# nfurnon/disco

Hardware: NVIDIA H100
Metric: beamformed frames/sec (16kHz, 512-pt STFT) (higher is better)
Workload: dtype f32 (c64 spectra, f32 SCM accumulation, f64 per-bin solve)

## Files before the change

### disco_b200/csrc/common.cuh

```cuda
#pragma once
#include <cuda_runtime.h>
#include <stdint.h>

#define DISCO_DEV __device__ __forceinline__

namespace disco {

DISCO_DEV float2 fadd2(float2 a, float2 b) { return make_float2(__fadd_rn(a.x, b.x), __fadd_rn(a.y, b.y)); }
DISCO_DEV float2 fmul2(float2 a, float2 b) { return make_float2(__fmul_rn(a.x, b.x), __fmul_rn(a.y, b.y)); }
DISCO_DEV float2 ffma2(float2 a, float2 b, float2 c) {
    return make_float2(__fmaf_rn(a.x, b.x, c.x), __fmaf_rn(a.y, b.y, c.y));
}

DISCO_DEV double solve_scale(double t) {
    if (!(t >= 2.2250738585072014e-308 && t <= 1.7976931348623157e308)) return 1.0;
    const int e = ((__double2hiint(t) >> 20) & 0x7ff) - 1023;
    return __hiloint2double((1023 - e) << 20, 0);
}

DISCO_DEV float2 cadd(float2 a, float2 b) { return fadd2(a, b); }
DISCO_DEV float2 csub(float2 a, float2 b) { return fadd2(a, make_float2(-b.x, -b.y)); }
DISCO_DEV float2 cmul(float2 a, float2 b) {
    const float2 t = fmul2(make_float2(-b.y, b.x), make_float2(a.y, a.y));
    return ffma2(b, make_float2(a.x, a.x), t);
}
DISCO_DEV float2 cmulc(float2 a, float2 b) {
    const float2 t = fmul2(make_float2(a.y, -a.x), make_float2(b.y, b.y));
    return ffma2(a, make_float2(b.x, b.x), t);
}
DISCO_DEV float2 cfma(float2 a, float2 b, float2 acc) {
    const float2 t = ffma2(b, make_float2(a.x, a.x), acc);
    return ffma2(make_float2(-b.y, b.x), make_float2(a.y, a.y), t);
}
DISCO_DEV float2 cfma_cj(float2 a, float2 b, float2 acc) {
    const float2 t = ffma2(b, make_float2(a.x, a.x), acc);
    return ffma2(make_float2(b.y, -b.x), make_float2(a.y, a.y), t);
}
DISCO_DEV float2 cscale(float2 a, float s) { return fmul2(a, make_float2(s, s)); }
DISCO_DEV float2 cconj(float2 a) { return make_float2(a.x, -a.y); }
DISCO_DEV float2 cfma_r(float s, float2 a, float2 acc) { return ffma2(make_float2(s, s), a, acc); }

template <int C>
DISCO_DEV void dual_filter(const float2 (&w1)[C], const float2 (&w2)[C], const float2 (&y)[C], int ref, float2& z,
                           float2& zn, float2& yf) {
    z = make_float2(0.f, 0.f);
    yf = make_float2(0.f, 0.f);
#pragma unroll
    for (int c = 0; c < C; ++c) {
        z = cfma_cj(w1[c], y[c], z);
        yf = cfma_cj(w2[c], y[c], yf);
    }
    float2 r = y[0];
#pragma unroll
    for (int c = 1; c < C; ++c)
        if (c == ref) r = y[c];
    zn = csub(r, z);
}

DISCO_DEV uint32_t smem_u32(const void* p) { return (uint32_t)__cvta_generic_to_shared(p); }

DISCO_DEV void mbar_init(uint64_t* bar, uint32_t count) {
    asm volatile("mbarrier.init.shared::cta.b64 [%0], %1;" ::"r"(smem_u32(bar)), "r"(count));
}
DISCO_DEV void mbar_expect_tx(uint64_t* bar, uint32_t bytes) {
    asm volatile("mbarrier.arrive.expect_tx.shared::cta.b64 _, [%0], %1;" ::"r"(smem_u32(bar)), "r"(bytes)
                 : "memory");
}
DISCO_DEV void mbar_arrive(uint64_t* bar) {
    asm volatile("mbarrier.arrive.shared::cta.b64 _, [%0];" ::"r"(smem_u32(bar)) : "memory");
}
DISCO_DEV void mbar_wait(uint64_t* bar, uint32_t parity) {
    const uint32_t addr = smem_u32(bar);
    uint32_t done;
    do {
        asm volatile(
            "{\n"
            ".reg .pred p;\n"
            "mbarrier.try_wait.parity.shared::cta.b64 p, [%1], %2, %3;\n"
            "selp.u32 %0, 1, 0, p;\n"
            "}\n"
            : "=r"(done)
            : "r"(addr), "r"(parity), "r"(20000u)
            : "memory");
    } while (!done);
}
DISCO_DEV void tma_load_1d(void* dst_smem, const void* src_gmem, uint32_t bytes, uint64_t* bar) {
    asm volatile(
        "cp.async.bulk.shared::cluster.global.mbarrier::complete_tx::bytes [%0], [%1], %2, [%3];" ::"r"(
            smem_u32(dst_smem)),
        "l"(src_gmem), "r"(bytes), "r"(smem_u32(bar))
        : "memory");
}
DISCO_DEV void named_bar_sync(int id, int nthreads) {
    asm volatile("bar.sync %0, %1;" ::"r"(id), "r"(nthreads) : "memory");
}
DISCO_DEV void fence_proxy_async() { asm volatile("fence.proxy.async.shared::cta;" ::: "memory"); }
DISCO_DEV void fence_mbar_init() { asm volatile("fence.mbarrier_init.release.cluster;" ::: "memory"); }

DISCO_DEV void st_stream(float2* p, float2 v) { __stcs(p, v); }
DISCO_DEV float ld_stream(const float* p) { return __ldcs(p); }
DISCO_DEV float2 ld_stream(const float2* p) { return __ldcs(p); }

}
```

### disco_b200/csrc/stft_scm.cu

```cuda
#include "common.cuh"
#include "kernels.h"
#include "stft_core.cuh"

namespace disco {

enum : int { OUT_Y = 0, OUT_NONE = 1, OUT_FILTER = 2, OUT_FILTER_FT = 3 };

template <int N, int C, int NM = 1, int OUT = OUT_Y>
struct StftCfg : StftJob<N> {
    static constexpr bool WIDE = C > 4;
    static constexpr int NSTG = 2;
    static constexpr int JOBS = 8;
    static constexpr int ITEMS = JOBS * StftJob<N>::NB;
    static constexpr int P = (C + 1) / 2;
    static constexpr int TT = ITEMS / P;
    static constexpr bool REALLOC = (N == 512) || (WIDE && N == 256);
    static constexpr bool DEAL = N == 512 && NM == 2 && C >= 3 && !WIDE;
    static constexpr int FFT_WARPS = DEAL ? 7 : (N == 512 && (WIDE || NM == 2)) ? 4 : 8;
    static constexpr int JPW = JOBS / FFT_WARPS;
    static constexpr int FFT_ARRIVALS = DEAL ? JOBS : FFT_WARPS;
    static constexpr int SCM_WARPS = N / 64;
    static constexpr int LEAD_WARPS = (REALLOC && !DEAL) ? 4 : 1;
    static constexpr int WARPS = LEAD_WARPS + FFT_WARPS + SCM_WARPS;
    static constexpr int THREADS = 32 * WARPS;
    static constexpr int SPEC = ITEMS * StftJob<N>::ROWP;
    static constexpr int SAMP = C * (TT + 1) * StftJob<N>::H;
    static constexpr int REG_LAUNCH = 16384 / ((WARPS + 3) / 4) / 32 / 8 * 8;
    static constexpr bool FILT = OUT == OUT_FILTER || OUT == OUT_FILTER_FT;
    static constexpr int REG_SCM = FILT ? 80 : WIDE ? 184 : ((N == 512 && NM == 2) ? 152 : 120);
    static constexpr int REG_FFT_CAP = 256;
    static constexpr int REG_ALLOC = (REG_LAUNCH > 255 ? 255 : REG_LAUNCH) * THREADS;
    static constexpr int REG_LEAD_OWN = FILT ? 56 : 32;
    static constexpr int REG_FFT_LEFT =
        DEAL ? (REG_ALLOC - 32 * SCM_WARPS * REG_SCM) / (32 * (LEAD_WARPS + FFT_WARPS)) / 8 * 8
             : (REG_ALLOC - 128 * REG_LEAD_OWN - 32 * SCM_WARPS * REG_SCM) / (32 * FFT_WARPS) / 8 * 8;
    static constexpr int REG_FFT = REG_FFT_LEFT < REG_FFT_CAP ? REG_FFT_LEFT : REG_FFT_CAP;
    static constexpr int REG_LEAD = DEAL ? REG_FFT : REG_LEAD_OWN;
    static constexpr int REG_SUM = DEAL ? 32 * (LEAD_WARPS + FFT_WARPS) * REG_FFT + 32 * SCM_WARPS * REG_SCM
                                        : 128 * REG_LEAD + 32 * FFT_WARPS * REG_FFT + 32 * SCM_WARPS * REG_SCM;
    static constexpr int FT_PITCH = 34;
    static constexpr int FT_STAGE = OUT == OUT_FILTER_FT ? SCM_WARPS * 8 * FT_PITCH : 0;
    static_assert(!REALLOC || (REG_LEAD >= 24 && REG_FFT >= 24), "setmaxnreg budgets start at 24");
    static_assert(!REALLOC || REG_SUM <= (REG_LAUNCH > 255 ? 255 : REG_LAUNCH) * THREADS,
                  "register budgets exceed the CTA's allocation");
    static_assert(!DEAL || (REALLOC && LEAD_WARPS + FFT_WARPS == 8 && WARPS == 16 && REG_LAUNCH == 128 &&
                            REG_FFT == 104 && REG_SUM == 65536),
                  "DEAL: loader + 7 FFT warps fill two warpgroups at 104 registers next to 8 SCM warps at 152");
    static_assert(DEAL || WIDE || NM != 2 || N != 512 || (FFT_WARPS == 4 && REG_SCM == 152 && REG_FFT == 176),
                  "two masks, 1-2 microphones at 512 points: 4 FFT warps at 176 registers next to SCM warps at 152");
    static_assert(!DEAL || JOBS >= FFT_WARPS, "DEAL: every FFT warp must run a job of every tile (the fill barrier)");
};

int stft_tile_frames(int n_fft, int C) { return (8 * (32 / (n_fft / 32))) / ((C + 1) / 2); }

template <int N, int C, int OUT = OUT_Y>
__host__ __device__ inline size_t smem_bytes() {
    using G = StftCfg<N, C, 1, OUT>;
    return G::NSTG * ((size_t)G::SPEC * sizeof(float2) + (size_t)G::SAMP * sizeof(float)) + (size_t)N * sizeof(float2) + 256 +
           64 * sizeof(float) + (size_t)G::FT_STAGE * sizeof(float2);
}

__device__ __forceinline__ long long range_lo(long long total, int b, int nb) { return total * b / nb; }

template <int R, int LAUNCH>
DISCO_DEV void set_maxnreg() {
    if constexpr (R > LAUNCH) {
        asm volatile("setmaxnreg.inc.sync.aligned.u32 %0;\n" ::"n"(R));
    } else if constexpr (R < LAUNCH) {
        asm volatile("setmaxnreg.dec.sync.aligned.u32 %0;\n" ::"n"(R));
    }
}

template <int C, int NM>
struct ScmAcc {
    static constexpr int NOFF = C * (C - 1) / 2;
    static constexpr int NO = NOFF > 0 ? NOFF : 1;
    float2 d[NM > 0 ? NM : 1][C];
    float2 os[NM > 0 ? NM : 1][NO];
    float2 on[NM > 0 ? NM : 1][NO];
    DISCO_DEV void reset() {
#pragma unroll
        for (int q = 0; q < NM; ++q) {
#pragma unroll
            for (int i = 0; i < C; ++i) d[q][i] = make_float2(0.f, 0.f);
#pragma unroll
            for (int i = 0; i < NOFF; ++i) os[q][i] = on[q][i] = make_float2(0.f, 0.f);
        }
    }
    DISCO_DEV void step(const float2 (&y)[C], const float (&m)[NM > 0 ? NM : 1]) {
        float2 ab[NM > 0 ? NM : 1];
#pragma unroll
        for (int q = 0; q < NM; ++q) {
            const float om = 1.f - m[q];
            ab[q] = make_float2(m[q] * m[q], om * om);
        }
        int o = 0;
#pragma unroll
        for (int i = 0; i < C; ++i) {
            const float dd = fmaf(y[i].x, y[i].x, y[i].y * y[i].y);
#pragma unroll
            for (int q = 0; q < NM; ++q) d[q][i] = ffma2(make_float2(dd, dd), ab[q], d[q][i]);
#pragma unroll
            for (int j = i + 1; j < C; ++j) {
                const float2 op = cmulc(y[i], y[j]);
#pragma unroll
                for (int q = 0; q < NM; ++q) {
                    os[q][o] = cfma_r(ab[q].x, op, os[q][o]);
                    on[q][o] = cfma_r(ab[q].y, op, on[q][o]);
                }
                ++o;
            }
        }
    }
    DISCO_DEV void flush(float* out, int F) const {
        int a = 0;
#pragma unroll
        for (int q = 0; q < NM; ++q) {
#pragma unroll
            for (int i = 0; i < C; ++i) out[(size_t)(a++) * F] = d[q][i].x;
#pragma unroll
            for (int i = 0; i < NOFF; ++i) {
                out[(size_t)(a++) * F] = os[q][i].x;
                out[(size_t)(a++) * F] = os[q][i].y;
            }
#pragma unroll
            for (int i = 0; i < C; ++i) out[(size_t)(a++) * F] = d[q][i].y;
#pragma unroll
            for (int i = 0; i < NOFF; ++i) {
                out[(size_t)(a++) * F] = on[q][i].x;
                out[(size_t)(a++) * F] = on[q][i].y;
            }
        }
    }
};

enum : int { RC_SAMP_FULL = 0, RC_SAMP_EMPTY = 1, RC_SPEC_FULL = 2, RC_SPEC_EMPTY = 3 };
enum : int { RC_ROLE_LOADER = 1, RC_ROLE_FFT = 2, RC_ROLE_SCM = 3 };
#ifdef DISCO_ROLE_CLOCKS
constexpr int RC_MAX_CTAS = 1024, RC_SLOTS = 8;
__device__ unsigned long long g_role_clocks[RC_MAX_CTAS * 32 * RC_SLOTS];
DISCO_DEV long long rc_clock() {
    long long t;
    asm volatile("mov.u64 %0, %%clock64;" : "=l"(t)::"memory");
    return t;
}
struct RoleClocks {
    long long t0, w[4] = {0, 0, 0, 0};
    int tiles = 0, jobs = 0;
    DISCO_DEV RoleClocks() : t0(rc_clock()) {}
    DISCO_DEV void wait(int k, uint64_t* bar, uint32_t parity) {
        const long long a = rc_clock();
        mbar_wait(bar, parity);
        w[k] += rc_clock() - a;
    }
    DISCO_DEV void tile() { ++tiles; }
    DISCO_DEV void job() { ++jobs; }
    DISCO_DEV void done(int role) {
        const long long t1 = rc_clock();
        if ((threadIdx.x & 31) != 0 || blockIdx.x >= RC_MAX_CTAS) return;
        unsigned long long* o = g_role_clocks + ((size_t)blockIdx.x * 32 + (threadIdx.x >> 5)) * RC_SLOTS;
        o[0] = role;
        o[1] = tiles;
        o[2] = jobs;
        o[3] = t1 - t0;
        for (int k = 0; k < 4; ++k) o[4 + k] = w[k];
    }
};
#else
struct RoleClocks {
    DISCO_DEV void wait(int, uint64_t* bar, uint32_t parity) { mbar_wait(bar, parity); }
    DISCO_DEV void tile() {}
    DISCO_DEV void job() {}
    DISCO_DEV void done(int) {}
};
#endif

template <int OUT>
struct StftParam {
    using type = StftArgs;
};
template <>
struct StftParam<OUT_FILTER> {
    using type = StftFilterArgs;
};
template <>
struct StftParam<OUT_FILTER_FT> {
    using type = StftFilterArgs;
};

template <int N, int C, int NM, int OUT>
__global__ void __launch_bounds__(StftCfg<N, C, NM, OUT>::THREADS, 1) stft_scm_kernel(typename StftParam<OUT>::type p) {
    using G = StftCfg<N, C, NM, OUT>;
    constexpr int RA = G::RA, NB = G::NB, H = G::H, F = G::F, ROWP = G::ROWP, P = G::P, TT = G::TT;
    constexpr int SAMP = G::SAMP;
    constexpr int NACC = NM * 2 * C * C;
    constexpr int NMX = NM > 0 ? NM : 1;
    constexpr bool SCM = NM > 0;
    constexpr bool STORE_Y = OUT == OUT_Y, FILT = G::FILT, FT = OUT == OUT_FILTER_FT;
    static_assert(!FILT || NM == 0, "the filter consumer accumulates no statistics");
    constexpr int MCAP = (G::REALLOC && G::REG_SCM >= 152 && !G::WIDE) ? 16 : 8;
    constexpr int MC = (TT * NM <= MCAP) ? TT : ((MCAP / NMX) < TT ? (MCAP / NMX) : TT);
    constexpr int NCH = (TT + MC - 1) / MC;

    extern __shared__ __align__(128) unsigned char smem_raw[];
    constexpr int NSTG = G::NSTG;
    float2* spec = reinterpret_cast<float2*>(smem_raw);
    float* samp = reinterpret_cast<float*>(spec + NSTG * G::SPEC);
    float2* tw = reinterpret_cast<float2*>(samp + NSTG * SAMP);
    uint64_t* bars = reinterpret_cast<uint64_t*>(tw + N);
    uint64_t* samp_full = bars;
    uint64_t* samp_empty = bars + NSTG;
    uint64_t* spec_full = bars + 2 * NSTG;
    uint64_t* spec_empty = bars + 3 * NSTG;
    float* nyq = reinterpret_cast<float*>(bars + 32);
    float2* ft_stage = reinterpret_cast<float2*>(nyq + 64);
    static_assert(4 * NSTG <= 32, "barrier area");
    static_assert(TT * C <= 64 && TT <= 32, "Nyquist staging");

    const int tid = threadIdx.x, lane = tid & 31, warp = tid >> 5;
    const int L = p.L, T = p.T;
    const int tiles_per_grp = (T + TT - 1) / TT;
    const long long total = (long long)p.n_grp * tiles_per_grp;
    const long long lo = range_lo(total, blockIdx.x, gridDim.x), hi = range_lo(total, blockIdx.x + 1, gridDim.x);
    const int n_it = (int)(hi - lo);
    if (n_it <= 0) return;

    for (int i = tid; i < N; i += blockDim.x) tw[i] = p.twiddle[i];
    if (tid == 0) {
        for (int s = 0; s < NSTG; ++s) {
            mbar_init(&samp_full[s], 1);
            mbar_init(&samp_empty[s], G::FFT_ARRIVALS);
            mbar_init(&spec_full[s], G::FFT_ARRIVALS);
            mbar_init(&spec_empty[s], G::SCM_WARPS + 1);
        }
        fence_mbar_init();
    }
    __syncthreads();

    auto tile_of = [&](int it, int& grp, int& t0) {
        const long long i = lo + it;
        grp = (int)(i / tiles_per_grp);
        t0 = (int)(i % tiles_per_grp) * TT;
    };
    auto seg_slot = [&](int grp) { return blockIdx.x - seg_slots(grp, tiles_per_grp, total, gridDim.x).first; };
    auto mask_at = [&](int q, int grp, int t, int f) {
        const float* m = q == 0 ? p.mask : p.mask2;
        return p.mask_ft ? m[((size_t)grp * F + f) * T + t] : m[((size_t)grp * T + t) * F + f];
    };

    constexpr int FFT_WARP0 = G::LEAD_WARPS;
    constexpr int SCM_WARP0 = G::LEAD_WARPS + G::FFT_WARPS;
    const bool is_fft = warp >= FFT_WARP0 && warp < FFT_WARP0 + G::FFT_WARPS;
    if constexpr (G::DEAL) {
        if (warp < SCM_WARP0) set_maxnreg<G::REG_FFT, G::REG_LAUNCH>();
    }
    if (warp < G::LEAD_WARPS) {
        if (G::REALLOC && !G::DEAL) set_maxnreg<G::REG_LEAD, G::REG_LAUNCH>();
        if (warp != 0) return;
        RoleClocks rc;
        auto load_tile = [&](int it) {
            int grp, t0;
            tile_of(it, grp, t0);
            const int nfr = min(TT, T - t0), s = it % NSTG, c_valid = min(C, p.n_sig - grp * C);
            rc.wait(RC_SAMP_EMPTY, &samp_empty[s], ((it / NSTG) & 1) ^ 1);
            const float* xg = p.x + (size_t)grp * C * L;
            float* dst = samp + s * SAMP;
            const int s0 = t0 * H - H;
            const int cnt = (nfr + 1) * H;
            const int k_lo = max(0, -s0), k_hi = min(cnt, L - s0);
            if (lane == 0) {
                if (p.use_tma && k_hi > k_lo) {
                    fence_proxy_async();
                    mbar_expect_tx(&samp_full[s], (uint32_t)(c_valid * (k_hi - k_lo) * sizeof(float)));
                    for (int c = 0; c < c_valid; ++c)
                        tma_load_1d(dst + c * (TT + 1) * H + k_lo, xg + (size_t)c * L + s0 + k_lo,
                                    (uint32_t)((k_hi - k_lo) * sizeof(float)), &samp_full[s]);
                } else {
                    mbar_arrive(&samp_full[s]);
                }
            }
        };
        constexpr int NP = C * (C + 1) / 2;
        constexpr int NSLOT = NP > 32 ? 2 : 1;
        int pi[NSLOT], pj[NSLOT], row[NSLOT];
#pragma unroll
        for (int u = 0; u < NSLOT; ++u) {
            const int pp = min(lane + 32 * u, NP - 1);
            if (pp < C) {
                pi[u] = pj[u] = pp;
                row[u] = pp;
            } else {
                int o = pp - C, i = 0, n = C - 1;
                while (o >= n) {
                    o -= n;
                    --n;
                    ++i;
                }
                pi[u] = i;
                pj[u] = i + 1 + o;
                row[u] = C + 2 * (pp - C);
            }
        }
        float as[NMX][NSLOT], an[NMX][NSLOT];
        auto nyq_reset = [&]() {
#pragma unroll
            for (int q = 0; q < NMX; ++q)
#pragma unroll
                for (int u = 0; u < NSLOT; ++u) as[q][u] = an[q][u] = 0.f;
        };
        nyq_reset();
        float2 nw1[FILT ? C : 1], nw2[FILT ? C : 1];
        int nw_grp = -1;
        for (int i = 0; i < NSTG - 1; ++i)
            if (i < n_it) load_tile(i);
        for (int it = 0; it < n_it; ++it) {
            if (it + NSTG - 1 < n_it) load_tile(it + NSTG - 1);
            int grp, t0;
            tile_of(it, grp, t0);
            const int nfr = min(TT, T - t0), s = it % NSTG, c_valid = min(C, p.n_sig - grp * C);
            if constexpr (FILT) {
                if (grp != nw_grp) {
#pragma unroll
                    for (int c = 0; c < C; ++c) {
                        nw1[c] = p.W1[((size_t)grp * F + F - 1) * C + c];
                        nw2[c] = p.W2[((size_t)grp * F + F - 1) * C + c];
                    }
                    nw_grp = grp;
                }
                rc.wait(RC_SPEC_FULL, &spec_full[s], (it / NSTG) & 1);
                if (lane < nfr) {
                    float2 y[C];
#pragma unroll
                    for (int c = 0; c < C; ++c) {
                        const float2 z = spec[s * G::SPEC + (size_t)(lane * P + c / 2) * ROWP + N / 2];
                        y[c] = make_float2(stft_nyquist(z, c & 1), 0.f);
                    }
                    float2 z, zn, yf;
                    dual_filter<C>(nw1, nw2, y, p.ref, z, zn, yf);
                    const size_t o = FT ? ((size_t)grp * F + F - 1) * T + t0 + lane : ((size_t)grp * T + t0 + lane) * F + (F - 1);
                    __stcs(p.z + o, z);
                    if (p.zn) __stcs(p.zn + o, zn);
                    __stcs(p.yf + o, yf);
                }
                __syncwarp();
                if (lane == 0) mbar_arrive(&spec_empty[s]);
            } else {
                float mq[NMX];
#pragma unroll
                for (int q = 0; q < NMX; ++q) mq[q] = (SCM && lane < nfr) ? mask_at(q, grp, t0 + lane, F - 1) : 0.f;
                rc.wait(RC_SPEC_FULL, &spec_full[s], (it / NSTG) & 1);
#pragma unroll
                for (int r = lane; r < TT * C; r += 32) {
                    const int tl_l = r / C, c_l = r % C;
                    float yv = 0.f;
                    if (tl_l < nfr && c_l < c_valid) {
                        const float2 z = spec[s * G::SPEC + (size_t)(tl_l * P + c_l / 2) * ROWP + N / 2];
                        yv = (c_l & 1) ? z.y + z.y : z.x + z.x;
                        if (STORE_Y) p.Y[(((size_t)grp * C + c_l) * T + t0 + tl_l) * F + (F - 1)] = make_float2(yv, 0.f);
                    }
                    nyq[r] = yv;
                }
                __syncwarp();
                if (lane == 0) mbar_arrive(&spec_empty[s]);
                if (SCM) {
#pragma unroll
                    for (int tl = 0; tl < TT; ++tl) {
                        if (tl < nfr) {
                            float pr[NSLOT];
#pragma unroll
                            for (int u = 0; u < NSLOT; ++u)
                                pr[u] = nyq[tl * C + pi[u]] * nyq[tl * C + pj[u]];
#pragma unroll
                            for (int q = 0; q < NM; ++q) {
                                const float m = __shfl_sync(0xffffffffu, mq[q], tl), om = 1.f - m;
                                const float a = m * m, b = om * om;
#pragma unroll
                                for (int u = 0; u < NSLOT; ++u) {
                                    as[q][u] = fmaf(a, pr[u], as[q][u]);
                                    an[q][u] = fmaf(b, pr[u], an[q][u]);
                                }
                            }
                        }
                    }
                    const bool seg_end = (it + 1 == n_it) || ((lo + it + 1) % tiles_per_grp == 0);
                    if (seg_end) {
                        float* out = p.part + ((size_t)grp * p.slots_per_grp + seg_slot(grp)) * NACC * F + (F - 1);
#pragma unroll
                        for (int u = 0; u < NSLOT; ++u) {
                            const int pp = lane + 32 * u;
                            if (pp < NP) {
#pragma unroll
                                for (int q = 0; q < NM; ++q) {
                                    float* os = out + (size_t)(q * 2 * C * C) * F;
                                    float* on = os + (size_t)(C * C) * F;
                                    os[(size_t)row[u] * F] = as[q][u];
                                    on[(size_t)row[u] * F] = an[q][u];
                                    if (pp >= C) {
                                        os[(size_t)(row[u] + 1) * F] = 0.f;
                                        on[(size_t)(row[u] + 1) * F] = 0.f;
                                    }
                                }
                            }
                        }
                        nyq_reset();
                    }
                }
                __syncwarp();
            }
            rc.tile();
        }
        rc.done(RC_ROLE_LOADER);
    } else if (is_fft) {
        if (G::REALLOC && !G::DEAL) set_maxnreg<G::REG_FFT, G::REG_LAUNCH>();
        const int wf = warp - FFT_WARP0, f0 = wf / G::FFT_WARPS, w = wf % G::FFT_WARPS;
        constexpr bool WINREG = (RA <= 16);
        float win[WINREG ? RA : 1];
        if (WINREG) {
#pragma unroll
            for (int j = 0; j < RA; ++j) win[j] = p.window[lane + 32 * j];
        }
        RoleClocks rc;
        struct FftTile {
            int s, nfr, c_valid;
            const float* sm;
            bool full;
        };
        auto enter_tile = [&](int it) {
            int grp, t0;
            tile_of(it, grp, t0);
            const int nfr = min(TT, T - t0), s = it % NSTG, c_valid = min(C, p.n_sig - grp * C);
            const uint32_t ph = (it / NSTG) & 1;
            const float* sm = samp + s * SAMP;
            rc.wait(RC_SAMP_FULL, &samp_full[s], ph);
            {
                const int s0 = t0 * H - H;
                const int cnt = (nfr + 1) * H;
                int k_lo = max(0, -s0), k_hi = min(cnt, L - s0);
                if (!p.use_tma || k_hi <= k_lo) k_lo = k_hi = 0;
                const int n_fill = cnt - (k_hi - k_lo);
                if (n_fill > 0) {
                    const float* xg = p.x + (size_t)grp * C * L;
                    float* dst = samp + s * SAMP;
                    named_bar_sync(1 + f0, 32 * G::FFT_WARPS);
                    for (int c = 0; c < c_valid; ++c)
#pragma unroll(G::DEAL ? 1 : 4)
                        for (int q = w * 32 + lane; q < n_fill; q += 32 * G::FFT_WARPS) {
                            const int k = q < k_lo ? q : q + (k_hi - k_lo);
                            const int sidx = reflect_index(s0 + k, L);
                            float v = 0.f;
                            if (sidx >= 0 && sidx < L) v = xg[(size_t)c * L + sidx];
                            dst[c * (TT + 1) * H + k] = v;
                        }
                    named_bar_sync(1 + f0, 32 * G::FFT_WARPS);
                }
            }
            rc.wait(RC_SPEC_EMPTY, &spec_empty[s], ph ^ 1);
            const bool full = (nfr == TT && c_valid == C && (C % 2 == 0) && (G::ITEMS % P == 0));
            return FftTile{s, nfr, c_valid, sm, full};
        };
        auto run_job = [&](const FftTile& tc, int jb, bool release) {
            const int s = tc.s, nfr = tc.nfr, c_valid = tc.c_valid;
            const float* sm = tc.sm;
            const bool full = tc.full;
            float2* job = spec + s * G::SPEC + (size_t)jb * NB * ROWP;
            constexpr bool TWREG = (RA <= 16);
            float2 twr[TWREG ? RA : 1];
            if (TWREG) {
#pragma unroll
                for (int k1 = 1; k1 < RA; ++k1) twr[k1] = tw[k1 * 32 + lane];
            }
#pragma unroll
            for (int q = 0; q < NB; ++q) {
                const int item = jb * NB + q;
                const int tl = item / P, pr = item % P;
                const int ca = 2 * pr, cb = 2 * pr + 1;
                const float* xa = sm + ca * (TT + 1) * H + tl * H + lane;
                const float* xb = sm + cb * (TT + 1) * H + tl * H + lane;
                float2 v[RA];
                if (full || (tl < nfr && cb < c_valid)) {
#pragma unroll
                    for (int j = 0; j < RA; ++j) {
                        const float wj = WINREG ? win[j] : p.window[lane + 32 * j];
                        v[j] = fmul2(make_float2(xa[32 * j], xb[32 * j]), make_float2(wj, wj));
                    }
                } else if (tl < nfr && ca < c_valid) {
#pragma unroll
                    for (int j = 0; j < RA; ++j) {
                        const float wj = WINREG ? win[j] : p.window[lane + 32 * j];
                        v[j] = make_float2(xa[32 * j] * wj, 0.f);
                    }
                } else {
#pragma unroll
                    for (int j = 0; j < RA; ++j) v[j] = make_float2(0.f, 0.f);
                }
                if (release && q == NB - 1) {
                    __syncwarp();
                    if (lane == 0) mbar_arrive(&samp_empty[s]);
                }
                stft_pass1<RA, TWREG>(v, job, q, lane, twr, tw);
            }
            stft_pass2<RA>(job, lane);
            rc.job();
        };
        if constexpr (G::DEAL) {
            FftTile tc{};
            int cur = -1;
#pragma unroll 1
            for (int j = w; j < n_it * G::JOBS; j += G::FFT_WARPS) {
                const int it = j / G::JOBS;
                if (it != cur) {
                    tc = enter_tile(it);
                    cur = it;
                    rc.tile();
                }
                run_job(tc, j % G::JOBS, true);
                __syncwarp();
                if (lane == 0) mbar_arrive(&spec_full[tc.s]);
            }
        } else {
            for (int it = f0; it < n_it; ++it) {
                const FftTile tc = enter_tile(it);
#pragma unroll 1
                for (int jj = 0; jj < G::JPW; ++jj) run_job(tc, w * G::JPW + jj, jj == G::JPW - 1);
                __syncwarp();
                if (lane == 0) mbar_arrive(&spec_full[tc.s]);
                rc.tile();
            }
        }
        rc.done(RC_ROLE_FFT);
    } else {
        if (G::REALLOC) set_maxnreg<G::REG_SCM, G::REG_LAUNCH>();
        const int f = (warp - SCM_WARP0) * 32 + lane;
        const int fn = (N - f) & (N - 1);
        RoleClocks rc;
        if constexpr (FILT) {
            float2 w1[C], w2[C];
            int w_grp = -1;
            for (int it = 0; it < n_it; ++it) {
                int grp, t0;
                tile_of(it, grp, t0);
                const int nfr = min(TT, T - t0), s = it % NSTG;
                if (grp != w_grp) {
#pragma unroll
                    for (int c = 0; c < C; ++c) {
                        w1[c] = p.W1[((size_t)grp * F + f) * C + c];
                        w2[c] = p.W2[((size_t)grp * F + f) * C + c];
                    }
                    w_grp = grp;
                }
                const float2* stage = spec + s * G::SPEC;
                auto point = [&](int tl, float2& z, float2& zn, float2& yf) {
                    float2 y[C];
#pragma unroll
                    for (int pr = 0; pr < P; ++pr) {
                        const float2* row = stage + (size_t)(tl * P + pr) * ROWP;
                        float2 ya, yb;
                        stft_unmix(row[f], row[fn], ya, yb);
                        y[2 * pr] = ya;
                        if (2 * pr + 1 < C) y[2 * pr + 1] = yb;
                    }
                    dual_filter<C>(w1, w2, y, p.ref, z, zn, yf);
                };
                rc.wait(RC_SPEC_FULL, &spec_full[s], (it / NSTG) & 1);
                if constexpr (!FT) {
                    const size_t o = ((size_t)grp * T + t0) * F + f;
#pragma unroll 8
                    for (int tl = 0; tl < TT; ++tl) {
                        if (tl < nfr) {
                            float2 z, zn, yf;
                            point(tl, z, zn, yf);
                            __stcs(p.z + o + (size_t)tl * F, z);
                            if (p.zn) __stcs(p.zn + o + (size_t)tl * F, zn);
                            __stcs(p.yf + o + (size_t)tl * F, yf);
                        }
                    }
                } else {
                    float2* st = ft_stage + (warp - SCM_WARP0) * 8 * G::FT_PITCH;
                    const int fw = (warp - SCM_WARP0) * 32, jl = lane & 7;
                    auto flush = [&](float2* out, int c8) {
                        __syncwarp();
                        if (c8 + jl < nfr) {
#pragma unroll
                            for (int k = 0; k < 8; ++k) {
                                const int i = (lane >> 3) + 4 * k;
                                __stcs(out + ((size_t)grp * F + fw + i) * T + t0 + c8 + jl, st[jl * G::FT_PITCH + i]);
                            }
                        }
                        __syncwarp();
                    };
#pragma unroll 1
                    for (int c8 = 0; c8 < nfr; c8 += 8) {
                        float2 znr[8], yfr[8];
#pragma unroll
                        for (int j = 0; j < 8; ++j) {
                            float2 z = make_float2(0.f, 0.f);
                            znr[j] = yfr[j] = z;
                            if (c8 + j < nfr) point(c8 + j, z, znr[j], yfr[j]);
                            st[j * G::FT_PITCH + lane] = z;
                        }
                        flush(p.z, c8);
                        if (p.zn) {
#pragma unroll
                            for (int j = 0; j < 8; ++j) st[j * G::FT_PITCH + lane] = znr[j];
                            flush(p.zn, c8);
                        }
#pragma unroll
                        for (int j = 0; j < 8; ++j) st[j * G::FT_PITCH + lane] = yfr[j];
                        flush(p.yf, c8);
                    }
                }
                __syncwarp();
                if (lane == 0) mbar_arrive(&spec_empty[s]);
                rc.tile();
            }
            rc.done(RC_ROLE_SCM);
            return;
        }
        ScmAcc<C, NM> acc;
        float mk[NMX][MC];
        const int m_st = p.mask_ft ? 1 : F;
        const size_t m_f = p.mask_ft ? (size_t)f * T : (size_t)f;
        auto load_mask = [&](int it, int ch) {
            if (it >= n_it) return;
            int grp, t0;
            tile_of(it, grp, t0);
            const size_t base = (size_t)grp * T * F + m_f + (size_t)(t0 + ch * MC) * m_st;
#pragma unroll
            for (int q = 0; q < NM; ++q) {
                const float* mb = (q == 0 ? p.mask : p.mask2) + base;
#pragma unroll
                for (int i = 0; i < MC; ++i)
                    mk[q][i] = (ch * MC + i < TT && t0 + ch * MC + i < T) ? mb[i * m_st] : 0.f;
            }
        };
        if (SCM) {
            acc.reset();
            load_mask(0, 0);
        }
        for (int it = 0; it < n_it; ++it) {
            int grp, t0;
            tile_of(it, grp, t0);
            const int nfr = min(TT, T - t0), s = it % NSTG, c_valid = min(C, p.n_sig - grp * C);
            const float2* stage = spec + s * G::SPEC;
            float2* ybase = p.Y + ((size_t)grp * C * T + t0) * F + f;
            const size_t cstride = (size_t)T * F;
            const bool full = (nfr == TT && c_valid == C);
#pragma unroll
            for (int ch = 0; ch < NCH; ++ch) {
                float mcur[NMX][MC];
#pragma unroll
                for (int q = 0; q < NMX; ++q)
#pragma unroll
                    for (int i = 0; i < MC; ++i) mcur[q][i] = SCM ? mk[q][i] : 0.f;
                if (SCM) {
                    if (ch + 1 < NCH)
                        load_mask(it, ch + 1);
                    else
                        load_mask(it + 1, 0);
                }
                if (ch == 0) rc.wait(RC_SPEC_FULL, &spec_full[s], (it / NSTG) & 1);
#pragma unroll
                for (int i = 0; i < MC; ++i) {
                    const int tl = ch * MC + i;
                    if (tl < TT && (full || tl < nfr)) {
                        float2 y[C];
#pragma unroll
                        for (int pr = 0; pr < P; ++pr) {
                            const float2* row = stage + (size_t)(tl * P + pr) * ROWP;
                            float2 ya, yb;
                            stft_unmix(row[f], row[fn], ya, yb);
                            y[2 * pr] = ya;
                            if (2 * pr + 1 < C) y[2 * pr + 1] = yb;
                        }
                        if (STORE_Y) {
#pragma unroll
                            for (int c = 0; c < C; ++c)
                                if (full || c < c_valid) __stcs(ybase + c * cstride + tl * F, y[c]);
                        }
                        if (SCM) {
                            float m[NMX];
#pragma unroll
                            for (int q = 0; q < NMX; ++q) m[q] = mcur[q][i];
                            acc.step(y, m);
                        }
                    }
                }
            }
            __syncwarp();
            if (lane == 0) mbar_arrive(&spec_empty[s]);
            const bool seg_end = (it + 1 == n_it) || ((lo + it + 1) % tiles_per_grp == 0);
            if (SCM && seg_end) {
                acc.flush(p.part + ((size_t)grp * p.slots_per_grp + seg_slot(grp)) * NACC * F + f, F);
                acc.reset();
            }
            rc.tile();
        }
        rc.done(RC_ROLE_SCM);
    }
}

template <int C>
__global__ void __launch_bounds__(288) scm_finalize_kernel(const float* __restrict__ part, float2* __restrict__ Rss,
                                                           float2* __restrict__ Rnn, int n_grp, int slots_per_grp,
                                                           int tiles_per_grp, int n_cta, int F, float inv_T, int n_set,
                                                           int set) {
    constexpr int NA = 2 * C * C;
    const int g = blockIdx.x;
    const long long total = (long long)n_grp * tiles_per_grp;
    const int n_slot = seg_slots(g, tiles_per_grp, total, n_cta).count();
    const size_t slot_stride = (size_t)n_set * NA * F;
    for (int f = threadIdx.x; f < F; f += blockDim.x) {
        const float* base = part + (size_t)g * slots_per_grp * slot_stride + (size_t)set * NA * F + f;
#pragma unroll 1
        for (int which = 0; which < 2; ++which) {
            float acc[C * C];
#pragma unroll
            for (int a = 0; a < C * C; ++a) acc[a] = 0.f;
            for (int sl = 0; sl < n_slot; ++sl) {
#pragma unroll
                for (int a = 0; a < C * C; ++a) acc[a] += __ldg(base + sl * slot_stride + (size_t)(which * C * C + a) * F);
            }
            float2* R = (which == 0 ? Rss : Rnn) + ((size_t)g * F + f) * C * C;
            int o = 0;
#pragma unroll
            for (int i = 0; i < C; ++i) {
                R[i * C + i] = make_float2(acc[i] * inv_T, 0.f);
#pragma unroll
                for (int j = i + 1; j < C; ++j) {
                    const float re = acc[C + 2 * o] * inv_T, im = acc[C + 2 * o + 1] * inv_T;
                    R[i * C + j] = make_float2(re, im);
                    R[j * C + i] = make_float2(re, -im);
                    ++o;
                }
            }
        }
    }
}

int stft_tiles_per_grp(int n_fft, int C, int T) {
    const int tt = stft_tile_frames(n_fft, C);
    return (T + tt - 1) / tt;
}

bool stft_scm_supported(int n_fft, int C, int n_mask) {
    if (C < 1 || C > 8 || n_mask < 0 || n_mask > 2) return false;
    if (n_fft != 256 && n_fft != 512 && n_fft != 1024) return false;
    if (C > 4 && (n_mask == 2 || n_fft == 1024)) return false;
    if (n_mask == 2 && n_fft == 1024) return false;
    if (n_mask == 0 && C > 4) return false;
    return true;
}

template <int N, int C, int NM, int OUT = OUT_Y>
static cudaError_t launch_one(const typename StftParam<OUT>::type& a, int n_cta, cudaStream_t st) {
    using G = StftCfg<N, C, NM, OUT>;
    auto kern = stft_scm_kernel<N, C, NM, OUT>;
    const size_t smem = smem_bytes<N, C, OUT>();
    cudaError_t e = cudaFuncSetAttribute(kern, cudaFuncAttributeMaxDynamicSharedMemorySize, (int)smem);
    if (e != cudaSuccess) return e;
    if (G::REALLOC) {
        cudaFuncAttributes fa;
        e = cudaFuncGetAttributes(&fa, kern);
        if (e != cudaSuccess) return e;
        if ((long long)fa.numRegs * G::THREADS < G::REG_SUM) return cudaErrorLaunchOutOfResources;
    }
    kern<<<n_cta, G::THREADS, smem, st>>>(a);
    return cudaGetLastError();
}

template <int N, int C>
static cudaError_t launch_nm(const StftArgs& a, int nm, int n_cta, cudaStream_t st) {
    if constexpr (C <= 4) {
        if (nm == 0) return launch_one<N, C, 0>(a, n_cta, st);
    }
    if (nm == 1) return launch_one<N, C, 1>(a, n_cta, st);
    if constexpr (C <= 4 && N <= 512) {
        if (nm == 2) return a.Y ? launch_one<N, C, 2>(a, n_cta, st) : launch_one<N, C, 2, OUT_NONE>(a, n_cta, st);
    }
    return cudaErrorInvalidValue;
}

template <int N>
static cudaError_t launch_c(const StftArgs& a, int C, int nm, int n_cta, cudaStream_t st) {
    switch (C) {
        case 1: return launch_nm<N, 1>(a, nm, n_cta, st);
        case 2: return launch_nm<N, 2>(a, nm, n_cta, st);
        case 3: return launch_nm<N, 3>(a, nm, n_cta, st);
        case 4: return launch_nm<N, 4>(a, nm, n_cta, st);
        default: break;
    }
    if constexpr (N <= 512) {
        switch (C) {
            case 5: return launch_nm<N, 5>(a, nm, n_cta, st);
            case 6: return launch_nm<N, 6>(a, nm, n_cta, st);
            case 7: return launch_nm<N, 7>(a, nm, n_cta, st);
            case 8: return launch_nm<N, 8>(a, nm, n_cta, st);
            default: break;
        }
    }
    return cudaErrorInvalidValue;
}

cudaError_t launch_stft_scm(const StftArgs& a, int n_fft, int C, int n_cta, int n_mask, cudaStream_t st) {
    if (!stft_scm_supported(n_fft, C, n_mask)) return cudaErrorInvalidValue;
    switch (n_fft) {
        case 256: return launch_c<256>(a, C, n_mask, n_cta, st);
        case 512: return launch_c<512>(a, C, n_mask, n_cta, st);
        case 1024: return launch_c<1024>(a, C, n_mask, n_cta, st);
        default: return cudaErrorInvalidValue;
    }
}

cudaError_t launch_stft_filter_dual(const StftFilterArgs& a, int n_fft, int C, int n_cta, cudaStream_t st) {
    if (!stft_scm_supported(n_fft, C, 2)) return cudaErrorInvalidValue;
#define DISCO_SFD(NN, CC)                                                                                  \
    if (n_fft == NN && C == CC)                                                                            \
        return a.out_ft ? launch_one<NN, CC, 0, OUT_FILTER_FT>(a, n_cta, st) : launch_one<NN, CC, 0, OUT_FILTER>(a, n_cta, st);
    DISCO_SFD(256, 1) DISCO_SFD(256, 2) DISCO_SFD(256, 3) DISCO_SFD(256, 4)
    DISCO_SFD(512, 1) DISCO_SFD(512, 2) DISCO_SFD(512, 3) DISCO_SFD(512, 4)
#undef DISCO_SFD
    return cudaErrorInvalidValue;
}

cudaError_t launch_scm_finalize(const float* part, float2* Rss, float2* Rnn, int n_grp, int slots_per_grp,
                                int tiles_per_grp, int n_cta, int C, int F, int T, int n_set, int set, cudaStream_t st) {
    const float inv_T = 1.0f / (float)T;
#define DISCO_FIN(CC)                                                                                              \
    case CC:                                                                                                       \
        scm_finalize_kernel<CC><<<n_grp, 288, 0, st>>>(part, Rss, Rnn, n_grp, slots_per_grp, tiles_per_grp, n_cta, \
                                                       F, inv_T, n_set, set);                                      \
        break;
    switch (C) {
        DISCO_FIN(1)
        DISCO_FIN(2)
        DISCO_FIN(3)
        DISCO_FIN(4)
        DISCO_FIN(5)
        DISCO_FIN(6)
        DISCO_FIN(7)
        DISCO_FIN(8)
        default: return cudaErrorInvalidValue;
    }
#undef DISCO_FIN
    return cudaGetLastError();
}

}

#ifdef DISCO_ROLE_CLOCKS
extern "C" __attribute__((visibility("default"))) void disco_role_clocks_layout(int* max_ctas, int* slots) {
    *max_ctas = disco::RC_MAX_CTAS;
    *slots = disco::RC_SLOTS;
}
extern "C" __attribute__((visibility("default"))) long long disco_role_clocks(void* dst, size_t bytes, int reset) {
    const size_t n = sizeof(disco::g_role_clocks) < bytes ? sizeof(disco::g_role_clocks) : bytes;
    if (cudaDeviceSynchronize() != cudaSuccess) return -1;
    if (n && cudaMemcpyFromSymbol(dst, disco::g_role_clocks, n) != cudaSuccess) return -1;
    if (reset) {
        void* a = nullptr;
        if (cudaGetSymbolAddress(&a, disco::g_role_clocks) != cudaSuccess ||
            cudaMemset(a, 0, sizeof(disco::g_role_clocks)) != cudaSuccess || cudaDeviceSynchronize() != cudaSuccess)
            return -1;
    }
    return (long long)n;
}
#endif
```

Baseline: 100.6 million.

## Poll loader barriers non-blockingly to interleave sample loads with Nyquist work

The loader warp no longer blocks on samp_empty before each load and then on spec_full before each Nyquist tile. It now spins with mbarrier.test_wait on both barriers and runs whichever is ready, so sample prefetch and Nyquist/SCM processing can interleave instead of serialising. Nyquist mask loads are hoisted to the previous iteration so they overlap the wait. The cost is busy polling with warp votes, which may take issue slots from co-resident warps, plus more complex control flow.

```diff
diff --git a/disco_b200/csrc/common.cuh b/disco_b200/csrc/common.cuh
--- a/disco_b200/csrc/common.cuh
+++ b/disco_b200/csrc/common.cuh
@@ -69,6 +69,19 @@
 DISCO_DEV void mbar_arrive(uint64_t* bar) {
     asm volatile("mbarrier.arrive.shared::cta.b64 _, [%0];" ::"r"(smem_u32(bar)) : "memory");
 }
+DISCO_DEV bool mbar_test(uint64_t* bar, uint32_t parity) {
+    uint32_t done;
+    asm volatile(
+        "{\n"
+        ".reg .pred p;\n"
+        "mbarrier.test_wait.parity.shared::cta.b64 p, [%1], %2;\n"
+        "selp.u32 %0, 1, 0, p;\n"
+        "}\n"
+        : "=r"(done)
+        : "r"(smem_u32(bar)), "r"(parity)
+        : "memory");
+    return done != 0;
+}
 DISCO_DEV void mbar_wait(uint64_t* bar, uint32_t parity) {
     const uint32_t addr = smem_u32(bar);
     uint32_t done;
diff --git a/disco_b200/csrc/stft_scm.cu b/disco_b200/csrc/stft_scm.cu
--- a/disco_b200/csrc/stft_scm.cu
+++ b/disco_b200/csrc/stft_scm.cu
@@ -153,6 +153,8 @@
         mbar_wait(bar, parity);
         w[k] += rc_clock() - a;
     }
+    DISCO_DEV long long now() { return rc_clock(); }
+    DISCO_DEV void add(int k, long long since) { w[k] += rc_clock() - since; }
     DISCO_DEV void tile() { ++tiles; }
     DISCO_DEV void job() { ++jobs; }
     DISCO_DEV void done(int role) {
@@ -169,6 +171,8 @@
 #else
 struct RoleClocks {
     DISCO_DEV void wait(int, uint64_t* bar, uint32_t parity) { mbar_wait(bar, parity); }
+    DISCO_DEV long long now() { return 0; }
+    DISCO_DEV void add(int, long long) {}
     DISCO_DEV void tile() {}
     DISCO_DEV void job() {}
     DISCO_DEV void done(int) {}
@@ -262,7 +266,6 @@
             int grp, t0;
             tile_of(it, grp, t0);
             const int nfr = min(TT, T - t0), s = it % NSTG, c_valid = min(C, p.n_sig - grp * C);
-            rc.wait(RC_SAMP_EMPTY, &samp_empty[s], ((it / NSTG) & 1) ^ 1);
             const float* xg = p.x + (size_t)grp * C * L;
             float* dst = samp + s * SAMP;
             const int s0 = t0 * H - H;
@@ -311,10 +314,16 @@
         nyq_reset();
         float2 nw1[FILT ? C : 1], nw2[FILT ? C : 1];
         int nw_grp = -1;
-        for (int i = 0; i < NSTG - 1; ++i)
-            if (i < n_it) load_tile(i);
-        for (int it = 0; it < n_it; ++it) {
-            if (it + NSTG - 1 < n_it) load_tile(it + NSTG - 1);
+        float mq[NMX];
+        auto load_nyq_mask = [&](int it) {
+            if (FILT || it >= n_it) return;
+            int grp, t0;
+            tile_of(it, grp, t0);
+            const int nfr = min(TT, T - t0);
+#pragma unroll
+            for (int q = 0; q < NMX; ++q) mq[q] = (SCM && lane < nfr) ? mask_at(q, grp, t0 + lane, F - 1) : 0.f;
+        };
+        auto nyq_tile = [&](int it) {
             int grp, t0;
             tile_of(it, grp, t0);
             const int nfr = min(TT, T - t0), s = it % NSTG, c_valid = min(C, p.n_sig - grp * C);
@@ -327,7 +336,6 @@
                     }
                     nw_grp = grp;
                 }
-                rc.wait(RC_SPEC_FULL, &spec_full[s], (it / NSTG) & 1);
                 if (lane < nfr) {
                     float2 y[C];
 #pragma unroll
@@ -345,10 +353,6 @@
                 __syncwarp();
                 if (lane == 0) mbar_arrive(&spec_empty[s]);
             } else {
-                float mq[NMX];
-#pragma unroll
-                for (int q = 0; q < NMX; ++q) mq[q] = (SCM && lane < nfr) ? mask_at(q, grp, t0 + lane, F - 1) : 0.f;
-                rc.wait(RC_SPEC_FULL, &spec_full[s], (it / NSTG) & 1);
 #pragma unroll
                 for (int r = lane; r < TT * C; r += 32) {
                     const int tl_l = r / C, c_l = r % C;
@@ -407,6 +411,23 @@
                 }
                 __syncwarp();
             }
+        };
+        load_nyq_mask(0);
+        int nl = 0;
+        for (int nt = 0; nt < n_it;) {
+            if (nl < n_it && (nl < NSTG || __all_sync(0xffffffffu, mbar_test(&samp_empty[nl % NSTG], ((nl / NSTG) & 1) ^ 1)))) {
+                load_tile(nl++);
+                continue;
+            }
+            const long long t_poll = rc.now();
+            if (nl == n_it)
+                rc.wait(RC_SPEC_FULL, &spec_full[nt % NSTG], (nt / NSTG) & 1);
+            else if (!__all_sync(0xffffffffu, mbar_test(&spec_full[nt % NSTG], (nt / NSTG) & 1))) {
+                rc.add(RC_SAMP_EMPTY, t_poll);
+                continue;
+            }
+            nyq_tile(nt);
+            load_nyq_mask(++nt);
             rc.tile();
         }
         rc.done(RC_ROLE_LOADER);
```

After: 100.3 million (median of 6 runs). No clear change (-0.3%).
